# hyungman/SpRay

Measured on AMD Instinct MI355X. Metric: Mrays/s (primary+shadow), 64-domain wavelets, 1024x1024 8spp, 1/2/4/8 GPU, higher is better.
Workload: dtype f32; 1 GPU; wavelets64 1024x1024x8spp PT primary+shadow, all 64 domains resident per GPU (configs[1]); primary_rays=8388608, parallelism=one GPU, the whole frame

## Files before the change

spray_amd/csrc/rt_device.h:

```cpp
#pragma once

#include <hip/hip_runtime.h>

#include <climits>
#include <cstdint>

#include "rt_common.h"
#include "rt_kernels.h"
#include "spray_rt.h"

namespace spray_rt {
namespace {

constexpr float kInf = __builtin_inff();
constexpr int32_t kNone = INT_MAX;
constexpr int32_t kNoChildRef = INT32_MIN;

inline unsigned grid_for(size_t M) { return unsigned((M + kBlock - 1) / kBlock); }

#define GAS __attribute__((address_space(1)))
template <typename T>
__device__ __forceinline__ const GAS T* gptr(const T* p) {
  return (const GAS T*)(p);
}
typedef float v4f __attribute__((ext_vector_type(4)));
__device__ __forceinline__ float4 ld4(const void* base, size_t i) {
  const v4f v = reinterpret_cast<const GAS v4f*>(gptr(base))[i];
  return make_float4(v.x, v.y, v.z, v.w);
}

#define CAS __attribute__((address_space(4)))
__device__ __forceinline__ void ld_node(const void* nodes, size_t nb, float4& n0, float4& n1,
                                        float4& n2, float4& n3) {
  n0 = ld4(nodes, nb);
  n1 = ld4(nodes, nb + 1);
  n2 = ld4(nodes, nb + 2);
  n3 = ld4(nodes, nb + 3);
}
__device__ __forceinline__ void ld_tri(const void* tris, uint32_t p, float4& a, float4& b,
                                       float4& c) {
  a = ld4(tris, 3 * size_t(p));
  b = ld4(tris, 3 * size_t(p) + 1);
  c = ld4(tris, 3 * size_t(p) + 2);
}

struct Ray {
  float ox, oy, oz;
  float dx, dy, dz;
  float ix, iy, iz;
  float olx, oly, olz;
  float ohx, ohy, ohz;
};

__device__ __forceinline__ void ray_axis(float o, float i, float& ol, float& oh) {
  const float oi = o * i;
  const float s = copysignf(0x1p-21f * fabsf(oi), i);
  ol = oi + s;
  oh = oi - s;
}

__device__ __forceinline__ float clamp_dir(float d) {
  return fabsf(d) < kDirClamp ? copysignf(kDirClamp, d) : d;
}

__device__ __forceinline__ Ray make_ray(float ox, float oy, float oz, float dx,
                                        float dy, float dz) {
  Ray r;
  r.ox = ox; r.oy = oy; r.oz = oz;
  r.dx = dx; r.dy = dy; r.dz = dz;
  r.ix = 1.0f / clamp_dir(dx);
  r.iy = 1.0f / clamp_dir(dy);
  r.iz = 1.0f / clamp_dir(dz);
  ray_axis(ox, r.ix, r.olx, r.ohx);
  ray_axis(oy, r.iy, r.oly, r.ohy);
  ray_axis(oz, r.iz, r.olz, r.ohz);
  return r;
}

__device__ __forceinline__ bool slab(const Ray& r, float lx, float ly, float lz,
                                     float hx, float hy, float hz, float tnear,
                                     float tfar, float& tenter) {
  float t0x = fmaf(lx, r.ix, -r.olx), t1x = fmaf(hx, r.ix, -r.ohx);
  float t0y = fmaf(ly, r.iy, -r.oly), t1y = fmaf(hy, r.iy, -r.ohy);
  float t0z = fmaf(lz, r.iz, -r.olz), t1z = fmaf(hz, r.iz, -r.ohz);
  float tmin = fmaxf(fmaxf(fminf(t0x, t1x), fminf(t0y, t1y)),
                     fmaxf(fminf(t0z, t1z), tnear));
  float tmax = fminf(fminf(fmaxf(t0x, t1x), fmaxf(t0y, t1y)),
                     fminf(fmaxf(t0z, t1z), tfar * kTfarSlack));
  tenter = tmin;
  return tmin <= tmax;
}

__device__ __forceinline__ bool tri_test(const Ray& r, float tnear, float4 a,
                                         float4 b, float4 c, float& t,
                                         float& u, float& v) {
  const float cx = a.x - r.ox, cy = a.y - r.oy, cz = a.z - r.oz;
  const float rx = fmaf(r.dy, cz, -(r.dz * cy));
  const float ry = fmaf(r.dz, cx, -(r.dx * cz));
  const float rz = fmaf(r.dx, cy, -(r.dy * cx));
  const float den = fmaf(c.w, r.dz, fmaf(c.z, r.dy, c.y * r.dx));
  const float absden = fabsf(den);
  float U = fmaf(rz, c.x, fmaf(ry, b.w, rx * b.z));
  float V = fmaf(rz, b.y, fmaf(ry, b.x, rx * a.w));
  float T = fmaf(c.w, cz, fmaf(c.z, cy, c.y * cx));
  if (den < 0.0f) {
    U = -U;
    V = -V;
    T = -T;
  }
  if (!(den != 0.0f && U >= 0.0f && V >= 0.0f && U + V <= absden)) return false;
  const float tt = T / absden;
  if (!(tt > tnear)) return false;
  t = tt;
  u = U / absden;
  v = V / absden;
  return true;
}

struct DRay {
  float ox, oy, oz, ix, iy, iz;
};
__device__ __forceinline__ DRay make_dray(float ox, float oy, float oz,
                                          float dx, float dy, float dz) {
  DRay r;
  r.ox = ox; r.oy = oy; r.oz = oz;
  r.ix = 1.0f / dx;
  r.iy = 1.0f / dy;
  r.iz = 1.0f / dz;
  return r;
}
__device__ __forceinline__ bool aabb_ref6(float lx, float ly, float lz, float hx,
                                          float hy, float hz, const DRay& r,
                                          float& tmin_out) {
  const bool sx = r.ix < 0.0f, sy = r.iy < 0.0f, sz = r.iz < 0.0f;
  float tmin = ((sx ? hx : lx) - r.ox) * r.ix;
  float tmax = ((sx ? lx : hx) - r.ox) * r.ix;
  const float tymin = ((sy ? hy : ly) - r.oy) * r.iy;
  const float tymax = ((sy ? ly : hy) - r.oy) * r.iy;
  if ((tmin > tymax) || (tymin > tmax)) return false;
  if (tymin > tmin) tmin = tymin;
  if (tymax < tmax) tmax = tymax;
  const float tzmin = ((sz ? hz : lz) - r.oz) * r.iz;
  const float tzmax = ((sz ? lz : hz) - r.oz) * r.iz;
  if ((tmin > tzmax) || (tzmin > tmax)) return false;
  if (tzmin > tmin) tmin = tzmin;
  if (tzmax < tmax) tmax = tzmax;
  tmin_out = tmin;
  return (tmin < kInf) && (tmax > kRayEpsilon);
}
__device__ __forceinline__ bool aabb_ref(const float* box, const DRay& r,
                                         float& tmin_out) {
  return aabb_ref6(box[0], box[1], box[2], box[3], box[4], box[5], r, tmin_out);
}

struct Best {
  float t;
  uint32_t prim;
  uint32_t leaf;
};

template <bool ANY, bool COUNT>
__device__ __forceinline__ bool trace_tree(const void* nodes, const void* tris,
                                           const uint32_t* prims_, const Ray& r,
                                           float tnear, float tfar_any,
                                           Best& best, int32_t* stk,
                                           unsigned& nnode, unsigned& ntri) {
  const GAS uint32_t* __restrict__ prims = gptr(prims_);
  int sp = 0;
  int32_t cur = 0;
  for (;;) {
    const size_t nb = 4 * size_t(cur);
    float4 n0, n1, n2, n3;
    ld_node(nodes, nb, n0, n1, n2, n3);
    if (COUNT) ++nnode;
    const float tcut = ANY ? tfar_any : best.t;
    float tl, tr;
    const bool hl = slab(r, n0.x, n0.y, n0.z, n0.w, n1.x, n1.y, tnear, tcut, tl);
    const bool hr = slab(r, n1.z, n1.w, n2.x, n2.y, n2.z, n2.w, tnear, tcut, tr);
    int32_t c0 = __float_as_int(n3.x), c1 = __float_as_int(n3.y);
    bool h0 = hl, h1 = hr;
    if (hl && hr && tr < tl) {
      const int32_t x = c0;
      c0 = c1;
      c1 = x;
    } else if (!hl && hr) {
      c0 = c1;
      h0 = true;
      h1 = false;
    }
    int32_t next = kNone;
#pragma unroll
    for (int k = 0; k < 2; ++k) {
      const int32_t c = k == 0 ? c0 : c1;
      const bool h = k == 0 ? h0 : h1;
      if (!h) continue;
      if (c < 0) {
        const uint32_t enc = ~uint32_t(c);
        const uint32_t first = enc >> 2, cnt = (enc & 3u) + 1u;
        for (uint32_t q = 0; q < cnt; ++q) {
          const uint32_t p = first + q;
          float4 a, b, cc;
          ld_tri(tris, p, a, b, cc);
          if (COUNT) ++ntri;
          float t, u, v;
          if (!tri_test(r, tnear, a, b, cc, t, u, v)) continue;
          if (ANY) {
            if (t <= tfar_any) return true;
          } else {
            const uint32_t pid = prims[p];
            if (t < best.t || (t == best.t && pid < best.prim)) {
              best.t = t;
              best.prim = pid;
              best.leaf = p;
            }
          }
        }
      } else if (next == kNone) {
        next = c;
      } else {
        stk[sp * kBlock] = c;
        ++sp;
      }
    }
    if (next == kNone) {
      if (sp == 0) break;
      --sp;
      next = stk[sp * kBlock];
    }
    cur = next;
  }
  return false;
}

__device__ __forceinline__ float q_lo(float w) { return float(__float_as_uint(w) & 0xFFFFu); }
__device__ __forceinline__ float q_hi(float w) { return float(__float_as_uint(w) >> 16); }

struct QRay {
  float ix, iy, iz;
  float olx, oly, olz;
  float ohx, ohy, ohz;
};

__device__ __forceinline__ void q_axis(float base, float scale, float ix, float oix, float& qix,
                                       float& ol, float& oh) {
  const float o = -fmaf(base, ix, -oix);
  qix = scale * ix;
  const float ex = 0x1p-20f * ((fabsf(oix) + fabsf(o)) + 65536.0f * fabsf(qix));
  const float sx = copysignf(ex, ix);
  ol = o + sx;
  oh = o - sx;
}

__device__ __forceinline__ bool slab_q(const QRay& r, float lx, float ly, float lz, float hx,
                                       float hy, float hz, float tnear, float tfar,
                                       float& tenter) {
  float t0x = fmaf(lx, r.ix, -r.olx), t1x = fmaf(hx, r.ix, -r.ohx);
  float t0y = fmaf(ly, r.iy, -r.oly), t1y = fmaf(hy, r.iy, -r.ohy);
  float t0z = fmaf(lz, r.iz, -r.olz), t1z = fmaf(hz, r.iz, -r.ohz);
  float tmin = fmaxf(fmaxf(fminf(t0x, t1x), fminf(t0y, t1y)),
                     fmaxf(fminf(t0z, t1z), tnear));
  float tmax = fminf(fminf(fmaxf(t0x, t1x), fmaxf(t0y, t1y)),
                     fminf(fmaxf(t0z, t1z), tfar * kTfarSlack));
  tenter = tmin;
  return tmin <= tmax;
}

__device__ __forceinline__ bool occluded_tree_ww(const void* nodes, const void* tris,
                                                 const Ray& r, float tnear, float tfar,
                                                 int32_t* stk) {
  int sp = 0;
  int32_t cur = 0;
  int32_t leaf = kNone;
  for (;;) {
    while (cur >= 0 && cur != kNone) {
      float tl, tr;
      float4 n0, n1, n2, n3;
      ld_node(nodes, 4 * size_t(cur), n0, n1, n2, n3);
      const bool hl = slab(r, n0.x, n0.y, n0.z, n0.w, n1.x, n1.y, tnear, tfar, tl);
      const bool hr = slab(r, n1.z, n1.w, n2.x, n2.y, n2.z, n2.w, tnear, tfar, tr);
      int32_t c0 = __float_as_int(n3.x);
      int32_t c1 = __float_as_int(n3.y);
      if (hl && hr && tr < tl) {
        const int32_t x = c0;
        c0 = c1;
        c1 = x;
      }
      if (hl && hr) {
        stk[sp * kBlock] = c1;
        ++sp;
        cur = c0;
      } else if (hl || hr) {
        cur = hl ? c0 : c1;
      } else {
        cur = sp ? stk[--sp * kBlock] : kNone;
      }
      if (cur < 0 && leaf == kNone) {
        leaf = cur;
        cur = sp ? stk[--sp * kBlock] : kNone;
      }
      if (__ballot(leaf == kNone) == 0) break;
    }
    while (leaf != kNone) {
      const uint32_t enc = ~uint32_t(leaf);
      const uint32_t first = enc >> 2, cnt = (enc & 3u) + 1u;
      for (uint32_t q = 0; q < cnt; ++q) {
        float4 a, b, c;
        ld_tri(tris, first + q, a, b, c);
        float t, u, v;
        if (tri_test(r, tnear, a, b, c, t, u, v) && t <= tfar) return true;
      }
      leaf = kNone;
      if (cur < 0) {
        leaf = cur;
        cur = sp ? stk[--sp * kBlock] : kNone;
      }
    }
    if (cur == kNone) return false;
  }
}

template <int STK>
__device__ __forceinline__ bool occluded_tree_q4(const void* nodes, const void* tris,
                                                 const Ray& r, float tnear, float tfar,
                                                 int32_t* stk) {
  const char* nbytes = static_cast<const char*>(nodes);
  QRay qr;
  {
    const float4 base = ld4(nbytes - sizeof(QGrid), 0);
    const float4 scale = ld4(nbytes - sizeof(QGrid), 1);
    q_axis(base.x, scale.x, r.ix, r.ox * r.ix, qr.ix, qr.olx, qr.ohx);
    q_axis(base.y, scale.y, r.iy, r.oy * r.iy, qr.iy, qr.oly, qr.ohy);
    q_axis(base.z, scale.z, r.iz, r.oz * r.iz, qr.iz, qr.olz, qr.ohz);
  }
  constexpr int kOvf = kQ4Stack > STK ? kQ4Stack - STK : 1;
  int32_t ovf[kOvf];
  int sp = 0;
  auto push = [&](int32_t v) {
    if (STK >= kQ4Stack || sp < STK)
      stk[sp * kBlock] = v;
    else
      ovf[sp - STK] = v;
    ++sp;
  };
  auto pop = [&]() -> int32_t {
    if (sp == 0) return kNone;
    --sp;
    return (STK >= kQ4Stack || sp < STK) ? stk[sp * kBlock] : ovf[sp - STK];
  };
  int32_t cur = 0;
  int32_t leaf = kNone;
  for (;;) {
    while (cur >= 0 && cur != kNone) {
      const char* qp = nbytes - 128 - 64 * size_t(cur);
      const float4 a = ld4(qp, 0), b = ld4(qp, 1), c = ld4(qp, 2), d = ld4(qp, 3);
      const int32_t ref[4] = {__float_as_int(d.x), __float_as_int(d.y), __float_as_int(d.z),
                              __float_as_int(d.w)};
      float t[4];
      bool h[4];
      h[0] = slab_q(qr, q_lo(a.x), q_hi(a.x), q_lo(a.y), q_hi(a.y), q_lo(a.z), q_hi(a.z),
                    tnear, tfar, t[0]);
      h[1] = slab_q(qr, q_lo(a.w), q_hi(a.w), q_lo(b.x), q_hi(b.x), q_lo(b.y), q_hi(b.y),
                    tnear, tfar, t[1]);
      h[2] = slab_q(qr, q_lo(b.z), q_hi(b.z), q_lo(b.w), q_hi(b.w), q_lo(c.x), q_hi(c.x),
                    tnear, tfar, t[2]);
      h[3] = slab_q(qr, q_lo(c.y), q_hi(c.y), q_lo(c.z), q_hi(c.z), q_lo(c.w), q_hi(c.w),
                    tnear, tfar, t[3]);
      int32_t next = kNone;
      float tn = kInf;
#pragma unroll
      for (int k = 0; k < 4; ++k) {
        if (!h[k] || ref[k] == kNoChildRef) continue;
        if (next == kNone || t[k] < tn) {
          if (next != kNone) push(next);
          next = ref[k];
          tn = t[k];
        } else {
          push(ref[k]);
        }
      }
      cur = next != kNone ? next : pop();
      if (cur < 0 && leaf == kNone) {
        leaf = cur;
        cur = pop();
      }
      if (__ballot(leaf == kNone) == 0) break;
    }
    while (leaf != kNone) {
      const uint32_t enc = ~uint32_t(leaf);
      const uint32_t first = enc >> 2, cnt = (enc & 3u) + 1u;
      for (uint32_t q = 0; q < cnt; ++q) {
        float4 a, b, c;
        ld_tri(tris, first + q, a, b, c);
        float t, u, v;
// ... 301 lines not shown
```

spray_amd/csrc/rt_kernels.hip:

```cpp
#include <hip/hip_runtime.h>

#include <type_traits>

#include <hipcub/block/block_reduce.hpp>
#include <hipcub/block/block_scan.hpp>

#include <climits>
#include <cstdint>

#include "cam_device.h"
#include "rt_device.h"
#include "shade_device.h"

namespace spray_rt {
namespace {

#ifndef SPRAY_CHUNK_CH
#define SPRAY_CHUNK_CH 256
#endif
#ifndef SPRAY_CHUNK_AH
#define SPRAY_CHUNK_AH 128
#endif
#ifndef SPRAY_PERSIST_CH
#define SPRAY_PERSIST_CH 1
#endif
#ifndef SPRAY_PERSIST_AH
#define SPRAY_PERSIST_AH 0
#endif
constexpr size_t kPersistAhRays = size_t(16) << 20;

#ifndef SPRAY_AH_WW
#define SPRAY_AH_WW 1
#endif
#ifndef SPRAY_AH_QNODES
#define SPRAY_AH_QNODES 1
#endif
#ifndef SPRAY_WAVES_CH
#define SPRAY_WAVES_CH 6
#endif
#ifndef SPRAY_WAVES_KEYED
#define SPRAY_WAVES_KEYED 6
#endif
#ifndef SPRAY_WAVES_SHADOW
#define SPRAY_WAVES_SHADOW 6
#endif
#ifndef SPRAY_WAVES_AH
#define SPRAY_WAVES_AH 1
#endif
#ifndef SPRAY_AOGEN_LSTK
#define SPRAY_AOGEN_LSTK 8
#endif
#ifndef SPRAY_WAVES_AOGEN
#define SPRAY_WAVES_AOGEN 8
#endif

__device__ __forceinline__ int find_segment(const size_t* off, int nseg,
                                            size_t i) {
  int lo = 0, hi = nseg - 1;
  while (lo < hi) {
    const int mid = (lo + hi + 1) >> 1;
    if (off[mid] <= i)
      lo = mid;
    else
      hi = mid - 1;
  }
  return lo;
}

__global__ __launch_bounds__(kBlock) void k_rtc_intersect(
    const SlotDesc* __restrict__ slots, const int* __restrict__ seg_slot,
    const size_t* __restrict__ seg_off, int nseg, char* __restrict__ rays,
    size_t stride, size_t M) {
  __shared__ int32_t stack[kStack * kBlock];
  const size_t i = size_t(blockIdx.x) * kBlock + threadIdx.x;
  if (i >= M) return;
  const int seg = nseg == 1 ? 0 : find_segment(seg_off, nseg, i);
  const int slot = seg_slot[seg];
  const SlotDesc s = slots[slot];
  char* rec = rays + i * stride;
  const float* f = reinterpret_cast<const float*>(rec);
  const Ray r = make_ray(f[0], f[1], f[2], f[4], f[5], f[6]);
  const float tnear = f[8];
  Best best{f[9], 0xFFFFFFFFu, 0u};
  unsigned a = 0, b = 0;
  if (s.nnodes)
    trace_slot<false, false>(s, r, tnear, 0.f, best, stack + threadIdx.x, a, b);
  if (best.prim == 0xFFFFFFFFu) return;
  float hu, hv;
  const float4 c = hit_uv(s, r, tnear, best.leaf, hu, hv);
  uint32_t color;
  float nsx, nsy, nsz;
  epilogue(s, best.prim, hu, hv, color, nsx, nsy, nsz);
  float* o = reinterpret_cast<float*>(rec);
  uint32_t* ou = reinterpret_cast<uint32_t*>(rec);
  o[9] = best.t;
  o[12] = c.y;
  o[13] = c.z;
  o[14] = c.w;
  ou[15] = color;
  o[16] = hu;
  o[17] = hv;
  ou[18] = 0u;
  ou[19] = best.prim;
  o[21] = nsx;
  o[22] = nsy;
  o[23] = nsz;
}

__global__ __launch_bounds__(kBlock) void k_rtc_update(
    const SlotDesc* __restrict__ slots, const int* __restrict__ seg_slot,
    const size_t* __restrict__ seg_off, int nseg, char* __restrict__ rays,
    size_t stride, size_t M) {
  const size_t i = size_t(blockIdx.x) * kBlock + threadIdx.x;
  if (i >= M) return;
  const int seg = nseg == 1 ? 0 : find_segment(seg_off, nseg, i);
  const SlotDesc s = slots[seg_slot[seg]];
  char* rec = rays + i * stride;
  uint32_t* ou = reinterpret_cast<uint32_t*>(rec);
  float* o = reinterpret_cast<float*>(rec);
  if (ou[18] == 0xFFFFFFFFu || ou[19] >= s.ntris) return;
  uint32_t color;
  float nsx, nsy, nsz;
  epilogue(s, ou[19], o[16], o[17], color, nsx, nsy, nsz);
  ou[15] = color;
  o[21] = nsx;
  o[22] = nsy;
  o[23] = nsz;
}

__global__ __launch_bounds__(kBlock) void k_rtc_occluded(
    const SlotDesc* __restrict__ slots, const int* __restrict__ seg_slot,
    const size_t* __restrict__ seg_off, int nseg, char* __restrict__ rays,
    size_t stride, size_t M) {
  __shared__ int32_t stack[kStack * kBlock];
  const size_t i = size_t(blockIdx.x) * kBlock + threadIdx.x;
  if (i >= M) return;
  const int seg = nseg == 1 ? 0 : find_segment(seg_off, nseg, i);
  const SlotDesc s = slots[seg_slot[seg]];
  char* rec = rays + i * stride;
  const float* f = reinterpret_cast<const float*>(rec);
  const Ray r = make_ray(f[0], f[1], f[2], f[4], f[5], f[6]);
  Best best{0.f, 0u, 0u};
  unsigned a = 0, b = 0;
  if (s.nnodes &&
      trace_slot<true, false>(s, r, f[8], f[9], best, stack + threadIdx.x, a, b))
    reinterpret_cast<uint32_t*>(rec)[18] = 0u;
}

__global__ __launch_bounds__(kBlock) void k_domains(
    const float* __restrict__ boxes, int ndom, const float* __restrict__ org,
    const float* __restrict__ dir, size_t M, int* __restrict__ ids,
    float* __restrict__ ts, int* __restrict__ counts, int maxhits) {
  const size_t i = size_t(blockIdx.x) * kBlock + threadIdx.x;
  if (i >= M) return;
  const DRay r = make_dray(org[3 * i], org[3 * i + 1], org[3 * i + 2],
                           dir[3 * i], dir[3 * i + 1], dir[3 * i + 2]);
  float pt = -kInf;
  int pid = -1;
  int n = 0;
  for (; n < maxhits; ++n) {
    float bt = kInf;
    int bid = -1;
    for (int b = 0; b < ndom; ++b) {
      float tm;
      if (!aabb_ref(boxes + 6 * b, r, tm)) continue;
      const bool after = tm > pt || (tm == pt && b > pid);
      if (!after) continue;
      if (bid < 0 || tm < bt) {
        bt = tm;
        bid = b;
      }
    }
    if (bid < 0) break;
    ids[i * maxhits + n] = bid;
    ts[i * maxhits + n] = bt;
    pt = bt;
    pid = bid;
  }
  counts[i] = n;
}


struct SceneArgs {
  const SlotDesc* slots;
  const int* dom2slot;
  const DomTrav* domtrav;
  const float* boxes;
  int ndom;
  const BvhNode* tlas;
  int ntlas;
  const spray_rt_ray* rays;
  size_t M;
  const uint32_t* d_count;
  spray_rt_hit* hits;
  uint8_t* occ;
  unsigned long long* counters;
  uint32_t* heads;
  int persist;
  int heads_ready;
  int count_ready;
  ShadePt shade;
  spray_rt_ray* sh_out;
  uint8_t* sh_valid;
  uint32_t* sh_count;
  float4* sw;
  const uint32_t* idx;
  uint64_t* keys;
  const uint8_t* valid;
  const uint32_t* ao_pairs;
  const float4* ao_rec;
  const float4* ao_lv;
  int ao_ns;
  uint32_t* ao_fields;
  int ao_fb;
  uint32_t* tkeys;
  const uint32_t* tmin;
  size_t nrays;
  CamTable cam_tab;
  Cam cam;
  int cam_w, cam_spp;
  int direct_res;
};

#ifndef SPRAY_NT_IO
#define SPRAY_NT_IO 1
#endif
#ifndef SPRAY_HIT_TRANSPOSE
#define SPRAY_HIT_TRANSPOSE 1
#endif
#ifndef SPRAY_RAY_PREFETCH
#define SPRAY_RAY_PREFETCH 1
#endif
#ifndef SPRAY_GLDS_AUX
#define SPRAY_GLDS_AUX 0
#endif
typedef __attribute__((address_space(1))) const void* glds_src_t;
typedef __attribute__((address_space(3))) void* glds_dst_t;
#ifndef SPRAY_NT_IO_LANE
#define SPRAY_NT_IO_LANE 1
#endif

constexpr int kEpiNone = 0;
constexpr int kEpiSpawn = 1;
constexpr int kEpiKeys = 2;
constexpr int kEpiShadow = 3;
constexpr int kEpiShadowFrame = 4;
constexpr int kEpiAoGen = 5;
constexpr int kEpiAoGenF = 8;
constexpr bool ao_epi(int e) { return e == kEpiAoGen || e == kEpiAoGenF; }
constexpr int kEpiKeysShade = 6;
constexpr int kEpiShadowGen = 7;
constexpr bool rep_epi(int e) { return e == kEpiKeysShade || e == kEpiShadowGen; }

__device__ __host__ __forceinline__ size_t band_size(size_t M) {
  return (((M + kQueues - 1) / kQueues) + 63) / 64 * 64;
}

__device__ __forceinline__ void wave_lds_sync() {
  __builtin_amdgcn_fence(__ATOMIC_RELEASE, "wavefront");
  __builtin_amdgcn_wave_barrier();
  __builtin_amdgcn_fence(__ATOMIC_ACQUIRE, "wavefront");
}

struct AoSrc {
  float4 op, n4, x4, y4, l4;
};
__device__ __forceinline__ AoSrc ao_load(const SceneArgs& A, uint32_t pr) {
  const uint32_t i = pr >> 5, l = pr & 31u;
  const float4* rec = A.ao_rec + 4 * size_t(i);
  AoSrc o;
  o.op = rec[0];
  o.n4 = rec[1];
  o.x4 = rec[2];
  o.y4 = rec[3];
  o.l4 = A.ao_lv[size_t(__float_as_uint(o.op.w)) * uint32_t(A.ao_ns) + l];
  return o;
}
__device__ __forceinline__ void ao_ray(const AoSrc& o, v4f& a, v4f& b) {
  const float N[3] = {o.n4.x, o.n4.y, o.n4.z}, ax[3] = {o.x4.x, o.x4.y, o.x4.z},
              ay[3] = {o.y4.x, o.y4.y, o.y4.z};
  const float lv[3] = {o.l4.x, o.l4.y, o.l4.z};
  float w[3], pdf;
  hemisphere_apply(lv, N, ax, ay, w, pdf);
  a = v4f{o.op.x, o.op.y, o.op.z, kRayEpsilon};
  b = v4f{w[0], w[1], w[2], kInf};
}
__device__ __forceinline__ void ao_gen(const SceneArgs& A, size_t k, v4f& a, v4f& b) {
  ao_ray(ao_load(A, A.ao_pairs[k]), a, b);
}
__device__ __forceinline__ void ao_field(const SceneArgs& A, size_t k) {
  const uint32_t pr = A.ao_pairs[k];
  const size_t pos = size_t(pr >> 5) * uint32_t(A.ao_ns) + (pr & 31u);
  const uint32_t per = 32u / uint32_t(A.ao_fb);
  atomicOr(A.ao_fields + pos / per, 1u << (uint32_t(pos % per) * uint32_t(A.ao_fb)));
}

__device__ __forceinline__ bool ao_own(const AoSrc& o, const float* sbox, const float* spad,
                                       const float* sun, const uint8_t* sres, int nres) {
  v4f a, b;
  ao_ray(o, a, b);
  const Ray r = make_ray(a.x, a.y, a.z, b.x, b.y, b.z);
  float tm;
  if (!slab(r, sun[0], sun[1], sun[2], sun[3], sun[4], sun[5], 0.f, kInf, tm)) return false;
  for (int q = 0; q < nres; ++q) {
    const int d = int(sres[q]);
    const float* pb = spad + 6 * d;
    if (!slab(r, pb[0], pb[1], pb[2], pb[3], pb[4], pb[5], 0.f, kInf, tm)) continue;
    const DRay dr = make_dray(a.x, a.y, a.z, b.x, b.y, b.z);
    if (aabb_ref(sbox + 6 * d, dr, tm)) return true;
  }
  return false;
}

template <int W, bool ANY, bool COUNT, int EPI, int STK>
__device__ __forceinline__ void scene_ray(const SceneArgs& A, size_t i,
                                          const float4* stl, const float* sbox,
                                          const float4* sdom, int32_t* stk, int32_t* wstk,
                                          unsigned& nnode, unsigned& ntri,
                                          unsigned& nvisit, bool& spawn, float* pos,
                                          float* wi, const float* rin = nullptr) {
  constexpr bool kKeysL = EPI == kEpiKeys || EPI == kEpiKeysShade;
  const SlotDesc* __restrict__ slots = A.slots;
  const int* __restrict__ dom2slot = A.dom2slot;
  const int ntlas = A.ntlas;
  spray_rt_hit* __restrict__ hits = A.hits;
  uint8_t* __restrict__ occ = A.occ;
  {
    v4f a, b;
    if (ao_epi(EPI)) {
      ao_gen(A, i, a, b);
    } else if (rin) {
      a = v4f{rin[0], rin[1], rin[2], kRayEpsilon};
      b = v4f{rin[3], rin[4], rin[5], kInf};
    } else {
      const v4f* rp = reinterpret_cast<const v4f*>(A.rays + i);
      if (SPRAY_NT_IO_LANE) {
        a = __builtin_nontemporal_load(rp);
        b = __builtin_nontemporal_load(rp + 1);
      } else {
        a = rp[0];
        b = rp[1];
      }
    }
    const float4 o4 = make_float4(a.x, a.y, a.z, a.w), d4 = make_float4(b.x, b.y, b.z, b.w);
    const Ray r = make_ray(o4.x, o4.y, o4.z, d4.x, d4.y, d4.z);
    uint64_t m[W];
#pragma unroll
    for (int w = 0; w < W; ++w) m[w] = 0;
    tlas_mask_wave<W>(stl, ntlas, wstk, r, o4, d4, m);
    Best best{ANY ? 0.f : d4.w, 0xFFFFFFFFu, 0xFFFFFFFFu};
    int best_dom = -1;
    uint32_t it = 0, best_it = 0;
    bool occluded = false;
    for (;;) {
      float st = kInf;
      int sb = -1;
      bool any_left = false;
#pragma unroll
      for (int w = 0; w < W; ++w) any_left |= m[w] != 0;
      if (!any_left) break;
      {
        float dx = r.dx, dy = r.dy, dz = r.dz;
        asm volatile("" : "+v"(dx), "+v"(dy), "+v"(dz));
        const DRay dr = make_dray(r.ox, r.oy, r.oz, dx, dy, dz);
#pragma unroll
        for (int w = 0; w < W; ++w) {
          uint64_t bits = m[w];
          while (bits) {
            const int j = __ffsll((long long)bits) - 1;
            bits &= bits - 1;
            const int b = 64 * w + j;
            float tm;
            aabb_ref(sbox + 6 * b, dr, tm);
            if (sb < 0 || tm < st) {
              st = tm;
              sb = b;
            }
          }
        }
      }
#pragma unroll
      for (int w = 0; w < W; ++w)
        if (w == (sb >> 6)) m[w] &= ~(1ull << (sb & 63));
      const uint32_t pos_sb = it;
      if (kKeysL) ++it;
      const float4 dt = sdom[sb];
      const char* nodes = reinterpret_cast<const char*>(
          (uint64_t(__float_as_uint(dt.y)) << 32) | __float_as_uint(dt.x));
      if (!nodes) continue;
      const void* tris = nodes + __float_as_uint(dt.z);
      const uint32_t* prims = reinterpret_cast<const uint32_t*>(nodes + __float_as_uint(dt.w));
      if (COUNT) ++nvisit;
      if (ANY) {
        const bool o = (COUNT || SPRAY_AH_WW == 0)
                           ? trace_tree<true, COUNT>(nodes, tris, prims, r, o4.w, d4.w, best,
                                                     stk, nnode, ntri)
                           : SPRAY_AH_QNODES ? occluded_tree_q4<STK>(nodes, tris, r, o4.w, d4.w, stk)
                                             : occluded_tree_ww(nodes, tris, r, o4.w, d4.w, stk);
        if (o) {
          occluded = true;
          break;
        }
      } else {
        const uint32_t keep_prim = best.prim, keep_leaf = best.leaf;
        if (best_dom >= 0) best.prim = 0u;
        best.leaf = 0xFFFFFFFFu;
        trace_tree<false, COUNT>(nodes, tris, prims, r, o4.w, 0.f, best, stk, nnode,
                                 ntri);
        if (best.leaf != 0xFFFFFFFFu) {
          best_dom = sb;
          if (kKeysL) best_it = pos_sb;
        } else {
          best.prim = keep_prim;
          best.leaf = keep_leaf;
        }
      }
    }
    if (ANY) {
      occ[i] = occluded ? 1 : 0;
      if (EPI == kEpiAoGenF && occluded) ao_field(A, i);
    } else {
      float4 h0, h1, h2;
      if (best_dom < 0) {
        h0 = make_float4(kInf, 0.f, 0.f, __uint_as_float(0xFFFFFFFFu));
        h1 = make_float4(0.f, 0.f, 0.f, __uint_as_float(0u));
        h2 = make_float4(0.f, 0.f, 0.f, __int_as_float(-1));
      } else {
        const SlotDesc s = slots[dom2slot[best_dom]];
        float hu, hv;
        const float4 c = hit_uv(s, r, o4.w, best.leaf, hu, hv);
        uint32_t color;
        float nsx, nsy, nsz;
        epilogue(s, best.prim, hu, hv, color, nsx, nsy, nsz);
        h0 = make_float4(best.t, hu, hv, __uint_as_float(best.prim));
        h1 = make_float4(c.y, c.z, c.w, __uint_as_float(color));
        h2 = make_float4(nsx, nsy, nsz, __int_as_float(best_dom));
      }
      if (!((EPI == kEpiKeysShade || EPI == kEpiShadowFrame) && !hits)) {
        float4* hp = reinterpret_cast<float4*>(hits + i);
        hp[0] = h0;
        hp[1] = h1;
        hp[2] = h2;
      }
      if (kKeysL) {
        A.keys[i] = best_dom < 0 ? 0x7FFFFFFFFFFFFFFFull
                                 : (uint64_t(__float_as_uint(best.t)) << 32) |
                                       (uint64_t(best_it) << 16) | uint64_t(best_dom);
      }
      if (EPI == kEpiKeysShade) {
        A.tkeys[i] = best_dom >= 0 ? __float_as_uint(best.t) : 0xFFFFFFFFu;
        if (A.sh_valid) {
          bool sp = false;
          if (best_dom >= 0) {
            spray_rt_hit h;
            h.t = h0.x;
            h.color = __float_as_uint(h1.w);
            h.ns[0] = h2.x;
            h.ns[1] = h2.y;
            h.ns[2] = h2.z;
            const float d3[3] = {d4.x, d4.y, d4.z}, o3[3] = {o4.x, o4.y, o4.z};
            float L[3];
            sp = shade_pt_point(o3, d3, h, A.shade, pos, wi, L);
            if (sp) A.sw[i] = make_float4(L[0], L[1], L[2], 0.f);
          }
          A.sh_valid[i] = sp;
        }
      }
      if (EPI == kEpiSpawn && best_dom >= 0) {
        spray_rt_hit h;
        h.t = h0.x;
        h.color = __float_as_uint(h1.w);
        h.ns[0] = h2.x;
        h.ns[1] = h2.y;
        h.ns[2] = h2.z;
        h.domain = best_dom;
        spray_rt_ray ray;
        ray.org[0] = o4.x;
        ray.org[1] = o4.y;
        ray.org[2] = o4.z;
        ray.dir[0] = d4.x;
        ray.dir[1] = d4.y;
        ray.dir[2] = d4.z;
        spawn = shadow_pt(ray, h, A.shade, pos, wi);
      }
    }
  }
}

__device__ __forceinline__ uint32_t xcc_id() {
  uint32_t x;
  asm volatile("s_getreg_b32 %0, hwreg(HW_REG_XCC_ID, 0, 4)" : "=s"(x));
  return x;
}

__device__ __forceinline__ bool wave_coherent(const SceneArgs& A, size_t i, bool valid) {
  float dx = 0.f, dy = 0.f, dz = 0.f;
  if (valid) {
    const float4 d4 = reinterpret_cast<const float4*>(A.rays + i)[1];
    dx = d4.x;
    dy = d4.y;
    dz = d4.z;
  }
  const uint64_t vb = __ballot(valid);
  if (!vb) return true;
  const int lead = __ffsll((long long)vb) - 1;
  const float lx = __int_as_float(__builtin_amdgcn_readlane(__float_as_int(dx), lead));
  const float ly = __int_as_float(__builtin_amdgcn_readlane(__float_as_int(dy), lead));
  const float lz = __int_as_float(__builtin_amdgcn_readlane(__float_as_int(dz), lead));
  const float c = (dx * lx + dy * ly) + dz * lz;
  return __ballot(valid && !(c >= 0.99f)) == 0;
}

struct NoPost {
  __device__ void operator()() const {}
};
template <int W, bool ANY, int EPI, typename Post = NoPost>
__device__ __forceinline__ void scene_ray_packet(const SceneArgs& A, size_t i, bool valid,
                                                 const float4* stl, const float* sbox,
                                                 const float4* sdom, int32_t* wstk,
                                                 bool& spawn, float* pos, float* wi,
                                                 const float* rin = nullptr,
                                                 const Post& post = Post(),
                                                 const uint8_t* sres = nullptr, int nres = 0,
                                                 const float4* lray = nullptr) {
  const SlotDesc* __restrict__ slots = A.slots;
  const int* __restrict__ dom2slot = A.dom2slot;
  const int lane = threadIdx.x & 63;
  float4 o4 = make_float4(0.f, 0.f, 0.f, 0.f), d4 = make_float4(0.f, 0.f, 1.f, 0.f);
  if (lray) {
    asm volatile("s_waitcnt vmcnt(0)" ::: "memory");
    if (valid) {
      o4 = lray[lane];
      d4 = lray[64 + lane];
    }
  } else if (valid && rin) {
    o4 = make_float4(rin[0], rin[1], rin[2], kRayEpsilon);
    d4 = make_float4(rin[3], rin[4], rin[5], kInf);
  } else if (valid) {
    const v4f* rp = reinterpret_cast<const v4f*>(A.rays + i);
    v4f a, b;
    if (SPRAY_NT_IO) {
      a = __builtin_nontemporal_load(rp);
      b = __builtin_nontemporal_load(rp + 1);
    } else {
      a = rp[0];
      b = rp[1];
    }
    o4 = make_float4(a.x, a.y, a.z, a.w);
    d4 = make_float4(b.x, b.y, b.z, b.w);
  }
  const Ray r = make_ray(o4.x, o4.y, o4.z, d4.x, d4.y, d4.z);
  if constexpr (!std::is_same<Post, NoPost>::value) {
    asm volatile("" ::"v"(o4.x), "v"(d4.x));
    post();
  }
  uint64_t m[W];
#pragma unroll
  for (int w = 0; w < W; ++w) m[w] = 0;
  const bool direct = sres && A.direct_res;
  if (valid && direct) {
    const DRay dr = make_dray(o4.x, o4.y, o4.z, d4.x, d4.y, d4.z);
    for (int k = 0; k < nres; ++k) {
      const int d = int(sres[k]);
      float tm;
      if (aabb_ref(sbox + 6 * d, dr, tm)) {
#pragma unroll
        for (int w = 0; w < W; ++w)
          if (w == (d >> 6)) m[w] |= 1ull << (d & 63);
      }
    }
  } else if (valid) {
    tlas_mask_wave<W>(stl, A.ntlas, wstk, r, o4, d4, m);
  }
  constexpr bool kKeys = EPI == kEpiKeys || EPI == kEpiKeysShade;
  uint64_t m0[kKeys ? W : 1];
  if (kKeys) {
#pragma unroll
    for (int w = 0; w < W; ++w) m0[w] = m[w];
  }
  Best best{ANY ? 0.f : d4.w, 0xFFFFFFFFu, 0xFFFFFFFFu};
  int best_dom = -1;
  bool occluded = false;
  for (;;) {
    bool has = false;
#pragma unroll
    for (int w = 0; w < W; ++w) has |= m[w] != 0;
    const uint64_t hb = __ballot(has);
    if (!hb) break;
    const int lead = __ffsll((long long)hb) - 1;
    int sb = 0;
    if (lane == lead) {
      float st = kInf;
      sb = -1;
#pragma unroll
      for (int w = 0; w < W; ++w) {
        uint64_t bits = m[w];
        while (bits) {
          const int j = __ffsll((long long)bits) - 1;
          bits &= bits - 1;
          const int b = 64 * w + j;
          const float* bx = sbox + 6 * b;
          float tm;
          slab(r, bx[0], bx[1], bx[2], bx[3], bx[4], bx[5], -kInf, kInf, tm);
          if (sb < 0 || tm < st) {
            st = tm;
            sb = b;
          }
        }
      }
    }
    const int d = __builtin_amdgcn_readlane(sb, lead);
    bool act = false;
#pragma unroll
    for (int w = 0; w < W; ++w)
      if (w == (d >> 6)) {
        act = (m[w] >> (d & 63)) & 1ull;
        m[w] &= ~(1ull << (d & 63));
      }
    if (ANY) act = act && !occluded;
    if (!__ballot(act)) continue;
    const float4 dt = sdom[d];
    const uint32_t nlo = __builtin_amdgcn_readfirstlane(__float_as_uint(dt.x));
    const uint32_t nhi = __builtin_amdgcn_readfirstlane(__float_as_uint(dt.y));
    const uint64_t nodes = (uint64_t(nhi) << 32) | nlo;
    if (!nodes) continue;
    const uint64_t tris = nodes + __builtin_amdgcn_readfirstlane(__float_as_uint(dt.z));
    const uint64_t prims = nodes + __builtin_amdgcn_readfirstlane(__float_as_uint(dt.w));
    if (ANY) {
      bool hit = false;
      trace_tree_packet<true>(nodes, tris, prims, r, o4.w, d4.w, best, act, hit, wstk);
      if (hit) {
        occluded = true;
#pragma unroll
        for (int w = 0; w < W; ++w) m[w] = 0;
      }
    } else {
      Best loc{best_dom == -1 ? d4.w : best.t, 0xFFFFFFFFu, 0xFFFFFFFFu};
      bool hit = false;
      trace_tree_packet<false>(nodes, tris, prims, r, o4.w, 0.f, loc, act, hit, wstk);
      if (loc.leaf != 0xFFFFFFFFu) {
        bool take = best_dom == -1 || loc.t < best.t;
        if (!take && loc.t == best.t && best_dom >= 0) {
          const DRay dr = make_dray(o4.x, o4.y, o4.z, d4.x, d4.y, d4.z);
          float tmd, tme;
          aabb_ref(sbox + 6 * d, dr, tmd);
          aabb_ref(sbox + 6 * best_dom, dr, tme);
          take = tmd < tme || (tmd == tme && d < best_dom);
        }
        if (take) {
          best = loc;
          best_dom = d;
        }
      }
    }
  }
  if (ANY) {
    if (valid) A.occ[i] = occluded ? 1 : 0;
    if (EPI == kEpiAoGenF && valid && occluded) ao_field(A, i);
    return;
  }
  float4 h0, h1, h2;
  if (best_dom < 0) {
    h0 = make_float4(kInf, 0.f, 0.f, __uint_as_float(0xFFFFFFFFu));
    h1 = make_float4(0.f, 0.f, 0.f, __uint_as_float(0u));
    h2 = make_float4(0.f, 0.f, 0.f, __int_as_float(-1));
  } else {
    const SlotDesc s = slots[dom2slot[best_dom]];
    float hu, hv;
    const float4 c = hit_uv(s, r, o4.w, best.leaf, hu, hv);
    uint32_t color;
    float nsx, nsy, nsz;
    epilogue(s, best.prim, hu, hv, color, nsx, nsy, nsz);
    h0 = make_float4(best.t, hu, hv, __uint_as_float(best.prim));
    h1 = make_float4(c.y, c.z, c.w, __uint_as_float(color));
    h2 = make_float4(nsx, nsy, nsz, __int_as_float(best_dom));
  }
  const size_t i0 = size_t(__builtin_amdgcn_readfirstlane(uint32_t(i))) |
                    (size_t(__builtin_amdgcn_readfirstlane(uint32_t(i >> 32))) << 32);
  if ((EPI == kEpiKeysShade || EPI == kEpiShadowFrame) && !A.hits) {
  } else if (SPRAY_HIT_TRANSPOSE && (i0 & 63) == 0 &&
      __ballot(valid && i == i0 + size_t(lane)) == ~0ull) {
    const float hv[12] = {h0.x, h0.y, h0.z, h0.w, h1.x, h1.y, h1.z, h1.w,
                          h2.x, h2.y, h2.z, h2.w};
    v4f* wp = reinterpret_cast<v4f*>(A.hits + i0);
#pragma unroll
    for (int st = 0; st < 3; ++st) {
      const int g = 64 * st + lane;
      const int src = g / 3, ch = g - 3 * src;
      float o[4];
#pragma unroll
      for (int d = 0; d < 4; ++d) {
        const float a0 = __shfl(hv[d], src), a1 = __shfl(hv[4 + d], src),
                    a2 = __shfl(hv[8 + d], src);
        o[d] = ch == 0 ? a0 : (ch == 1 ? a1 : a2);
      }
      if (SPRAY_NT_IO)
        __builtin_nontemporal_store(v4f{o[0], o[1], o[2], o[3]}, wp + g);
      else
        wp[g] = v4f{o[0], o[1], o[2], o[3]};
    }
  } else if (valid) {
    if (SPRAY_NT_IO) {
      v4f* hp = reinterpret_cast<v4f*>(A.hits + i);
      __builtin_nontemporal_store(v4f{h0.x, h0.y, h0.z, h0.w}, hp);
      __builtin_nontemporal_store(v4f{h1.x, h1.y, h1.z, h1.w}, hp + 1);
      __builtin_nontemporal_store(v4f{h2.x, h2.y, h2.z, h2.w}, hp + 2);
    } else {
      float4* hp = reinterpret_cast<float4*>(A.hits + i);
      hp[0] = h0;
      hp[1] = h1;
      hp[2] = h2;
    }
  }
  if (!valid) return;
  if (kKeys) {
    uint64_t key = 0x7FFFFFFFFFFFFFFFull;
    if (best_dom >= 0 && direct) {
      key = (uint64_t(__float_as_uint(best.t)) << 32) | uint64_t(best_dom);
    } else if (best_dom >= 0) {
      const DRay dr = make_dray(o4.x, o4.y, o4.z, d4.x, d4.y, d4.z);
      float tb;
      aabb_ref(sbox + 6 * best_dom, dr, tb);
      uint32_t p = 0;
#pragma unroll
      for (int w = 0; w < W; ++w) {
        uint64_t bits = m0[w];
        while (bits) {
          const int j = __ffsll((long long)bits) - 1;
          bits &= bits - 1;
          const int b = 64 * w + j;
          float tm;
          aabb_ref(sbox + 6 * b, dr, tm);
          if (tm < tb || (tm == tb && b < best_dom)) ++p;
        }
      }
      key = (uint64_t(__float_as_uint(best.t)) << 32) | (uint64_t(p) << 16) |
            uint64_t(best_dom);
    }
    A.keys[i] = key;
    if (EPI == kEpiKeysShade) {
      A.tkeys[i] = best_dom >= 0 ? __float_as_uint(best.t) : 0xFFFFFFFFu;
      if (!A.sh_valid) return;
      bool sp = false;
      if (best_dom >= 0) {
        spray_rt_hit h;
        h.t = h0.x;
        h.color = __float_as_uint(h1.w);
        h.ns[0] = h2.x;
        h.ns[1] = h2.y;
        h.ns[2] = h2.z;
        const float d3[3] = {d4.x, d4.y, d4.z}, o3[3] = {o4.x, o4.y, o4.z};
        float L[3];
        sp = shade_pt_point(o3, d3, h, A.shade, pos, wi, L);
        if (sp) A.sw[i] = make_float4(L[0], L[1], L[2], 0.f);
      }
      A.sh_valid[i] = sp;
    }
  }
  if (EPI == kEpiShadowFrame && best_dom >= 0) {
    spray_rt_hit h;
    h.t = h0.x;
    h.color = __float_as_uint(h1.w);
    h.ns[0] = h2.x;
    h.ns[1] = h2.y;
    h.ns[2] = h2.z;
    const float d3[3] = {d4.x, d4.y, d4.z}, o3[3] = {o4.x, o4.y, o4.z};
    float L[3];
    spawn = shade_pt_point(o3, d3, h, A.shade, pos, wi, L);
    if (spawn) A.sw[i] = make_float4(L[0], L[1], L[2], 0.f);
  }
  if ((EPI == kEpiSpawn || EPI == kEpiShadow) && best_dom >= 0) {
    spray_rt_hit h;
    h.t = h0.x;
    h.color = __float_as_uint(h1.w);
    h.ns[0] = h2.x;
    h.ns[1] = h2.y;
    h.ns[2] = h2.z;
    h.domain = best_dom;
    spray_rt_ray ray;
    ray.org[0] = o4.x;
    ray.org[1] = o4.y;
    ray.org[2] = o4.z;
    ray.dir[0] = d4.x;
    ray.dir[1] = d4.y;
    ray.dir[2] = d4.z;
    spawn = shadow_pt(ray, h, A.shade, pos, wi);
  }
}

template <int EPI>
__device__ __forceinline__ bool rep_ray(const SceneArgs& A, size_t j, size_t i, bool ok, bool inb,
                                        size_t& at, float* r6, const float* sbox,
                                        const uint8_t* sres, int nres) {
  const bool cam = A.cam_tab.runs != nullptr;
  at = j;
  const auto miss = [&]() {
    if (EPI == kEpiKeysShade && !cam && inb) {
      A.keys[j] = 0x7FFFFFFFFFFFFFFFull;
      A.tkeys[j] = 0xFFFFFFFFu;
      if (A.sh_valid) A.sh_valid[j] = 0;
    }
    return false;
  };
  float o[3], d[3];
  if (cam) {
    if (!inb) return false;
    int x, y, s;
    cam_item(A.cam_tab, A.cam_spp, j, x, y, s, at);
    float fx, fy;
    insitu_jitter(A.cam_w, A.cam_spp, x, y, s, fx, fy);
    cam_dir(A.cam, fx, fy, d);
    o[0] = A.cam.p[0];
    o[1] = A.cam.p[1];
    o[2] = A.cam.p[2];
  } else {
    if (!ok) return miss();
    const float4* rp = reinterpret_cast<const float4*>(A.rays + i);
    const float4 o4 = rp[0], d4 = rp[1];
    o[0] = o4.x;
    o[1] = o4.y;
    o[2] = o4.z;
    d[0] = d4.x;
    d[1] = d4.y;
    d[2] = d4.z;
  }
  if (EPI == kEpiKeysShade) {
    r6[0] = o[0];
    r6[1] = o[1];
    r6[2] = o[2];
    r6[3] = d[0];
    r6[4] = d[1];
    r6[5] = d[2];
  } else {
    const uint32_t tb = A.tmin[at];
    if (tb == 0xFFFFFFFFu) return false;
    const float t = __uint_as_float(tb);
    r6[0] = d[0] * t + o[0];
    r6[1] = d[1] * t + o[1];
    r6[2] = d[2] * t + o[2];
    float w[3] = {A.shade.lp[0] - r6[0], A.shade.lp[1] - r6[1], A.shade.lp[2] - r6[2]};
    gnorm3(w);
    r6[3] = w[0];
    r6[4] = w[1];
    r6[5] = w[2];
  }
  const DRay dr = make_dray(r6[0], r6[1], r6[2], r6[3], r6[4], r6[5]);
  for (int k = 0; k < nres; ++k) {
    float tm;
    if (aabb_ref(sbox + 6 * int(sres[k]), dr, tm)) return true;
  }
  return miss();
}


__device__ __forceinline__ void store_shadow(const SceneArgs& A, bool active,
                                             bool flag, size_t i,
                                             const float* pos, const float* wi,
                                             uint32_t& wcount) {
  if (active) {
    A.sh_valid[i] = flag ? 1 : 0;
    if (flag) {
      float4* op = reinterpret_cast<float4*>(A.sh_out + i);
      op[0] = make_float4(pos[0], pos[1], pos[2], kRayEpsilon);
      op[1] = make_float4(wi[0], wi[1], wi[2], kInf);
    }
  }
  wcount += uint32_t(__popcll(__ballot(flag)));
}

#ifndef SPRAY_SHADOW_Q
#define SPRAY_SHADOW_Q 104
#endif
constexpr uint32_t kShadowQ = SPRAY_SHADOW_Q;
constexpr uint32_t kShadowT = kShadowQ - 64;
static_assert(kShadowQ > 64 && kShadowQ <= 128, "shadow queue capacity in (64, 128]");
struct ShadowQueue {
  float* ray;
  uint32_t* src;
  uint32_t n;
};

template <int W>
__device__ __forceinline__ void shadow_trace(const SceneArgs& A, const ShadowQueue& q,
                                             uint32_t cnt, const float4* stl, const float* sbox,
                                             const float4* sdom, int32_t* wstk) {
  const uint32_t lane = threadIdx.x & 63;
  const bool v = lane < cnt;
  const size_t s = v ? q.src[lane] : 0;
  bool f = false;
  float p[3], w[3];
  scene_ray_packet<W, true, kEpiNone>(A, s, v, stl, sbox, sdom, wstk, f, p, w, q.ray + 6 * lane);
}

template <int W>
__device__ __forceinline__ void shadow_push(const SceneArgs& A, ShadowQueue& q, bool active,
                                            bool flag, size_t i, const float* pos,
                                            const float* wi, const float4* stl,
                                            const float* sbox, const float4* sdom,
                                            int32_t* wstk, uint32_t& wcount) {
  const uint32_t lane = threadIdx.x & 63;
  if (active) A.sh_valid[i] = flag ? 1 : 0;
  const unsigned long long bal = __ballot(flag);
  if (!bal) return;
  wcount += uint32_t(__popcll(bal));
  if (flag) {
    const uint32_t k = q.n + uint32_t(__popcll(bal & ((1ull << lane) - 1ull)));
    float* e = q.ray + 6 * k;
    e[0] = pos[0];
    e[1] = pos[1];
    e[2] = pos[2];
    e[3] = wi[0];
    e[4] = wi[1];
    e[5] = wi[2];
    q.src[k] = uint32_t(i);
  }
  q.n += uint32_t(__popcll(bal));
  if (q.n < kShadowT) return;
  wave_lds_sync();
  const uint32_t cnt = q.n < 64 ? q.n : 64u;
  shadow_trace<W>(A, q, cnt, stl, sbox, sdom, wstk);
  const uint32_t rest = q.n - cnt;
  const bool mv = lane < rest;
  float e[6];
  uint32_t si = 0;
// ... 1624 lines not shown
```

Baseline: 14160 Mrays/s.

## Parallelize domain ordering across wave lanes and skip domains beyond current hit

Replaces the serial leader-lane loop that slab-tests every candidate domain box with a wave-parallel scheme. Each lane tests one box against the leader's broadcast ray, then a DPP wave-min and ballot pick the nearest domain. It also adds a per-lane cull (SPRAY_DOM_SKIP) that deactivates a ray for a domain whose entry distance exceeds its current closest hit. The code uses hand-written inline asm with s_nop hazard padding, which risks correctness on the target ISA and adds broadcast overhead when few domains remain.

```diff
diff --git a/spray_amd/csrc/rt_device.h b/spray_amd/csrc/rt_device.h
--- a/spray_amd/csrc/rt_device.h
+++ b/spray_amd/csrc/rt_device.h
@@ -89,6 +89,51 @@
                      fminf(fmaxf(t0z, t1z), tfar * kTfarSlack));
   tenter = tmin;
   return tmin <= tmax;
+}
+
+__device__ __forceinline__ float bcast_lane(float x, int l) {
+  return __int_as_float(__builtin_amdgcn_readlane(__float_as_int(x), l));
+}
+
+__device__ __forceinline__ void bcast_lane6(const float (&x)[6], int l, float (&s)[6]) {
+  asm volatile(
+      "s_nop 3\n\t"
+      "v_readlane_b32 %0, %6, %12\n\t"
+      "v_readlane_b32 %1, %7, %12\n\t"
+      "v_readlane_b32 %2, %8, %12\n\t"
+      "v_readlane_b32 %3, %9, %12\n\t"
+      "v_readlane_b32 %4, %10, %12\n\t"
+      "v_readlane_b32 %5, %11, %12\n\t"
+      "s_nop 1"
+      : "=&s"(s[0]), "=&s"(s[1]), "=&s"(s[2]), "=&s"(s[3]), "=&s"(s[4]), "=&s"(s[5])
+      : "v"(x[0]), "v"(x[1]), "v"(x[2]), "v"(x[3]), "v"(x[4]), "v"(x[5]), "s"(l));
+}
+
+__device__ __forceinline__ float lanes_or_inf(float x, uint64_t mask) {
+  float y;
+  asm("s_nop 1\n\t"
+      "v_mov_b32 %0, 0x7f800000\n\t"
+      "v_cndmask_b32_e64 %0, %0, %1, %2"
+      : "=&v"(y)
+      : "v"(x), "s"(mask));
+  return y;
+}
+
+__device__ __forceinline__ float wave_min(float x) {
+  asm("s_nop 1\n\t"
+      "v_min_f32_dpp %0, %0, %0 quad_perm:[1,0,3,2] row_mask:0xf bank_mask:0xf\n\t"
+      "s_nop 1\n\t"
+      "v_min_f32_dpp %0, %0, %0 quad_perm:[2,3,0,1] row_mask:0xf bank_mask:0xf\n\t"
+      "s_nop 1\n\t"
+      "v_min_f32_dpp %0, %0, %0 row_half_mirror row_mask:0xf bank_mask:0xf\n\t"
+      "s_nop 1\n\t"
+      "v_min_f32_dpp %0, %0, %0 row_mirror row_mask:0xf bank_mask:0xf\n\t"
+      "s_nop 1\n\t"
+      "v_min_f32_dpp %0, %0, %0 row_bcast:15 row_mask:0xa bank_mask:0xf\n\t"
+      "s_nop 1\n\t"
+      "v_min_f32_dpp %0, %0, %0 row_bcast:31 row_mask:0xc bank_mask:0xf"
+      : "+v"(x));
+  return __int_as_float(__builtin_amdgcn_readlane(__float_as_int(x), 63));
 }
 
 __device__ __forceinline__ bool tri_test(const Ray& r, float tnear, float4 a,
diff --git a/spray_amd/csrc/rt_kernels.hip b/spray_amd/csrc/rt_kernels.hip
--- a/spray_amd/csrc/rt_kernels.hip
+++ b/spray_amd/csrc/rt_kernels.hip
@@ -240,6 +240,10 @@
 #define SPRAY_NT_IO_LANE 1
 #endif
 
+#ifndef SPRAY_DOM_SKIP
+#define SPRAY_DOM_SKIP 1
+#endif
+
 constexpr int kEpiNone = 0;
 constexpr int kEpiSpawn = 1;
 constexpr int kEpiKeys = 2;
@@ -588,28 +592,53 @@
     const uint64_t hb = __ballot(has);
     if (!hb) break;
     const int lead = __ffsll((long long)hb) - 1;
-    int sb = 0;
-    if (lane == lead) {
-      float st = kInf;
-      sb = -1;
+    uint64_t lm[W];
+    int left = 0;
+#pragma unroll
+    for (int w = 0; w < W; ++w) {
+      lm[w] = uint64_t(uint32_t(__builtin_amdgcn_readlane(int(uint32_t(m[w])), lead))) |
+              (uint64_t(uint32_t(__builtin_amdgcn_readlane(int(uint32_t(m[w] >> 32)), lead))) << 32);
+      left += __popcll(lm[w]);
+    }
+    int d = 0;
+    if (left == 1) {
+#pragma unroll
+      for (int w = 0; w < W; ++w)
+        if (lm[w]) d = 64 * w + __ffsll((long long)lm[w]) - 1;
+    } else {
+      Ray rl;
+      rl.ix = bcast_lane(r.ix, lead);
+      rl.iy = bcast_lane(r.iy, lead);
+      rl.iz = bcast_lane(r.iz, lead);
+      const float no[6] = {-r.olx, -r.oly, -r.olz, -r.ohx, -r.ohy, -r.ohz};
+      float nl[6];
+      bcast_lane6(no, lead, nl);
+      rl.olx = -nl[0];
+      rl.oly = -nl[1];
+      rl.olz = -nl[2];
+      rl.ohx = -nl[3];
+      rl.ohy = -nl[4];
+      rl.ohz = -nl[5];
+      float tent[W];
+      int lj = lane;
+      asm volatile("" : "+v"(lj));
 #pragma unroll
       for (int w = 0; w < W; ++w) {
-        uint64_t bits = m[w];
-        while (bits) {
-          const int j = __ffsll((long long)bits) - 1;
-          bits &= bits - 1;
-          const int b = 64 * w + j;
-          const float* bx = sbox + 6 * b;
-          float tm;
-          slab(r, bx[0], bx[1], bx[2], bx[3], bx[4], bx[5], -kInf, kInf, tm);
-          if (sb < 0 || tm < st) {
-            st = tm;
-            sb = b;
-          }
-        }
-      }
-    }
-    const int d = __builtin_amdgcn_readlane(sb, lead);
+        const float* bx = sbox + 6 * (64 * w + lj);
+        float tm;
+        slab(rl, bx[0], bx[1], bx[2], bx[3], bx[4], bx[5], -kInf, kInf, tm);
+        tent[w] = lanes_or_inf(tm, lm[w]);
+      }
+      float tmin = tent[0];
+#pragma unroll
+      for (int w = 1; w < W; ++w) tmin = fminf(tmin, tent[w]);
+      tmin = wave_min(tmin);
+#pragma unroll
+      for (int w = W - 1; w >= 0; --w) {
+        const uint64_t eq = __ballot(tent[w] == tmin) & lm[w];
+        if (eq) d = 64 * w + __ffsll((long long)eq) - 1;
+      }
+    }
     bool act = false;
 #pragma unroll
     for (int w = 0; w < W; ++w)
@@ -618,8 +647,15 @@
         m[w] &= ~(1ull << (d & 63));
       }
     if (ANY) act = act && !occluded;
+    if (SPRAY_DOM_SKIP && !ANY) {
+      const float* bx = sbox + 6 * d;
+      float tm;
+      slab(r, bx[0], bx[1], bx[2], bx[3], bx[4], bx[5], -kInf, kInf, tm);
+      act = act && !(best_dom >= 0 && best.t > 0.f && tm > best.t * kTfarSlack);
+    }
     if (!__ballot(act)) continue;
     const float4 dt = sdom[d];
+    asm volatile("" ::"v"(dt.x), "v"(dt.y), "v"(dt.z), "v"(dt.w));
     const uint32_t nlo = __builtin_amdgcn_readfirstlane(__float_as_uint(dt.x));
     const uint32_t nhi = __builtin_amdgcn_readfirstlane(__float_as_uint(dt.y));
     const uint64_t nodes = (uint64_t(nhi) << 32) | nlo;
```

Result: no change. 14290 Mrays/s (median of 2 runs) (+1.0%).
